# MVME-HBUT/Faster-OreFSDet

Hardware: AMD Instinct MI355X
Metric: images/sec at 640x640 25-shot (eval FPS: model(inputs) + device sync per image, bs=1 per GPU) (higher is better)
Workload: dtype f32

## Files before the change

### faster-orefsdet_amd/csrc/ore_conv_internal.h

```cpp
#pragma once
#include "ore_common.h"

namespace oreconv {

struct Lvl { int orow0, irow0, H, W, Ho, Wo; };

struct ConvP {
    const float* in; int in_ld, in_coff;
    int B, Cin;
    int nlev; Lvl lv[4];
    const float* w;
    int Cout, Cout16, kh, kw, stride, pad, M, K;
    const float* scale; const float* shift; int ep_stride; int relu_cout;
    const float* in_mul; const float* in_add; int in_relu;
    const float* add; int add_ld, add_coff, add_H, add_W;
    float* out; int out_ld, out_coff;
    float* colsum;
    int splitk, steps_per_split, nchunks;
    float* ws; int* tile_cnt;
    int bf16;
    int xmap;
    int sb;
    const float* wino;
    size_t w_lstride;
// ... 69 lines not shown
    int kw_force[4] = {};
    int gs_force[2] = {};
    int gs_ns = 3;
    int xmap_force = -1;
    int kw_nw_force = 0;
    int wino_mode = 1;
    int ws_sb_mode = 1;
    int ws_s2_mode = 1;
    int rf_mode = 1;
    int rf_force[3] = {};
    int kd_mode = 1;
    int kd_force[4] = {};
    int gd_mode = 1;
    int gd_force[3] = {};
    int gd_dbg = 0;
    int igemm[5] = {};
};
extern ConvKnobs g_knobs;

using ConvPlan = ore_conv_plan_t;
ConvPlan conv_plan(const ConvP& p, int req_splitk, size_t workspace_floats);
bool conv_wino_covers(int Cout, int Cin);
int wino_level_blocks(const ConvP& p, int gy, int* blk0);

int launch_ws(const ConvP& p, const ConvPlan& pl, hipStream_t st);
int launch_patch(const ConvP& p, const ConvPlan& pl, hipStream_t st);
int launch_igemm(const ConvP& p, const ConvPlan& pl, hipStream_t st);
int launch_wino(const ConvP& p, const ConvPlan& pl, hipStream_t st);
int launch_gd(const ConvP& p, const ConvPlan& pl, hipStream_t st);
int launch_kd(const ConvP& p, const ConvPlan& pl, hipStream_t st);
// ... 10 lines not shown
```

### faster-orefsdet_amd/csrc/ore_conv_plan.cpp

```cpp
#include "ore_common.h"
#include "ore_conv_internal.h"

namespace oreconv {

ConvKnobs g_knobs;

namespace {

const ConvKnobs& K = g_knobs;

ConvPlan make_plan(int launcher, int bm, int bn, int b0, int b1, int b2, int b3, int gx, int gy, int xmap = 0, int splitk = 1, int sps = 0) {
    ConvPlan pl{};
    pl.launcher = launcher; pl.error = ORE_OK;
    pl.bm = bm; pl.bn = bn;
    pl.build[0] = b0; pl.build[1] = b1; pl.build[2] = b2; pl.build[3] = b3;
    pl.splitk = splitk; pl.steps_per_split = sps; pl.xmap = xmap;
    pl.gx = gx; pl.gy = gy;
    return pl;
}

ConvPlan none() { return ConvPlan{}; }

ConvPlan fail(int code) {
    ConvPlan pl{};
// ... 83 lines not shown
    if (c.kh != 3 || c.kw != 3 || c.stride != 1 || c.pad != 1 || c.in_mul || c.add || c.colsum) return none();
    if (c.Cout != c.Cout16 || !conv_wino_covers(c.Cout, c.Cin)) return none();
    if (c.out_ld % 4 != 0 || c.out_coff % 4 != 0 || ((uintptr_t)c.out & 15) != 0 || c.in_ld % 4 != 0 || c.in_coff % 4 != 0) return none();
    if (c.ep_stride % 4 != 0 || ((uintptr_t)c.scale & 15) != 0 || ((uintptr_t)c.shift & 15) != 0) return none();
    if (K.wino_mode != 2 && !c.wino_lstride && c.M < ((c.Cin == 64 || c.Cin == 128) ? 1500 : 3000)) return none();
    for (int l = 0; l < c.nlev; ++l)
        if ((long long)c.lv[l].H * c.lv[l].W * c.in_ld * 4 >= (long long)kOOB) return none();
    const int nb = patch_tiles(c, 4);
    if (nb >= (1 << 22)) return none();
    if (c.Cin == 80 || c.Cin == 96 || c.Cin == 112) {
        const int ncgb = c.Cin == 80 ? 3 : 2;
        const int gy = ceil_div(c.Cout16 / 16, ncgb);
        int gx = 256 / gy;
        if (gx > nb) gx = nb;
        if (gx < 1) gx = 1;
        return make_plan(ORE_LAUNCH_WINO_NU, 4, ncgb * 16, c.Cin, ncgb, 0, 0, gx, gy);
    }
    const int coutb = c.Cin == 64 ? 64 : 32;
    const int gy = c.Cout / coutb;
    int gx = 256 / gy;
    if (gx > nb) gx = nb;
    if (gx < 1) gx = 1;
    if (c.wino_lstride) gx = wino_level_blocks(c, gy, nullptr);
    return make_plan(ORE_LAUNCH_WINO, 4, coutb, c.Cin, 0, 0, 0, gx, gy);
}

bool gd_flat(const ConvP& p) { return p.nlev > 1 && p.kh == 1 && p.kw == 1 && p.stride == 1 && p.pad == 0; }

bool gd_applies(const ConvP& p) {
    if (p.sb || p.in_mul || p.in_add || p.in_relu || (p.nlev != 1 && !gd_flat(p)) || p.ep_stride || (p.add && p.nlev != 1)) return false;
    if (p.Cin % 16 != 0 || p.in_ld % 16 != 0 || p.kh != p.kw || (p.kh != 1 && p.kh != 3)) return false;
    if (p.M >= (1 << 22) || p.nchunks > kGdTab) return false;
    const long long in_rows = gd_flat(p) ? (long long)p.lv[0].irow0 + p.M : (long long)p.lv[0].irow0 + (long long)p.B * p.lv[0].H * p.lv[0].W;
    if (in_rows * p.in_ld * 4 >= (long long)kOOB - (1 << 24) || (long long)p.Cout16 * p.K * 4 >= (long long)kOOB) return false;
    if (p.add && (long long)p.B * p.add_H * p.add_W * p.add_ld * 4 >= (long long)kOOB) return false;
    return true;
}
// ... 309 lines not shown
    return fail(ORE_EINVAL);
}

}

bool conv_wino_covers(int Cout, int Cin) {
    if (Cout <= 0 || Cout % 16 != 0) return false;
    if (Cin == 64) return Cout % 64 == 0;
    if (Cin == 128) return Cout % 32 == 0;
    return Cin == 80 || Cin == 96 || Cin == 112;
}

int wino_level_blocks(const ConvP& c, int gy, int* blk0) {
    int nb[4];
    for (int l = 0; l < c.nlev; ++l) nb[l] = c.B * ceil_div(c.lv[l].W, 16) * ceil_div(c.lv[l].H, 4);
    const int G = 256 / gy > c.nlev ? 256 / gy : c.nlev;
    int R = 1;
    for (;; ++R) {
        int need = 0;
        for (int l = 0; l < c.nlev; ++l) need += ceil_div(nb[l], R);
        if (need <= G) break;
    }
    int gx = 0;
    for (int l = 0; l < c.nlev; ++l) { if (blk0) blk0[l] = gx; gx += ceil_div(nb[l], R); }
    if (blk0) blk0[c.nlev] = gx;
    return gx;
}

ConvPlan conv_plan(const ConvP& p, int req_splitk, size_t workspace_floats) {
    ConvPlan pl;
    if (p.w_lstride) {
// ... 37 lines not shown
    case -1: k.patch_mode = BN; k.igemm[0] = 0; break;
    case -2: k.kw_mode = BN; k.igemm[0] = 0; break;
    case -3: k.kw_force[0] = BN; k.kw_force[1] = WGM; k.kw_force[2] = WGN; k.kw_force[3] = WGK; break;
    case -4: k.gs_force[0] = BN; k.gs_force[1] = WGM; if (WGN > 0) k.gs_ns = WGN; break;
    case -5: k.xmap_force = BN; break;
    case -6: k.kw_nw_force = BN; break;
    case -7: k.wino_mode = BN; break;
    case -8: k.ws_sb_mode = BN; break;
    case -9: k.ws_s2_mode = BN; break;
    case -10: k.rf_mode = BN; break;
    case -11: k.rf_force[0] = BN; k.rf_force[1] = WGM; k.rf_force[2] = WGN; break;
    case -12: k.kd_mode = BN; break;
    case -13: k.kd_force[0] = BN; k.kd_force[1] = WGM; k.kd_force[2] = WGN; k.kd_force[3] = WGK; break;
    case -14: k.gd_mode = BN; break;
    case -15: k.gd_force[0] = BN; k.gd_force[1] = WGM; k.gd_force[2] = WGN; break;
    case -16: k.gd_dbg = BN; break;
    default: k.igemm[0] = BM; k.igemm[1] = BN; k.igemm[2] = WGM; k.igemm[3] = WGN; k.igemm[4] = WGK; break;
    }
    return ORE_OK;
}

extern "C" int ore_conv_reset_plan_overrides(void) {
    g_knobs = ConvKnobs{};
    return ORE_OK;
}
```

### faster-orefsdet_amd/csrc/ore_conv_wino.hip

```cpp
#include "ore_conv_desc.h"
#include "ore_conv_epilogue.h"
#include <algorithm>

namespace {
using namespace oreconv;

struct WinoP {
    const float* in; int in_ld, in_coff;
    int B, nlev; Lvl lv[4]; int bat0[5]; int nbx[4], nby[4];
    float inv_per[4], inv_nbx[4];
    const float* U; int Cout, Cout16;
    size_t u_lstride; int blk0[5];
    const float* scale; const float* shift; int ep_stride, relu_cout;
    float* out; int out_ld, out_coff;
    int nbat;
};

struct WinoImg { __amdgpu_buffer_rsrc_t rs; unsigned pix_bytes, row_bytes; int H, W; };
__device__ __forceinline__ WinoImg wino_image(const WinoP& p, int irow0, int H, int W, int b) {
    WinoImg im;
    im.pix_bytes = (unsigned)p.in_ld * 4u; im.row_bytes = (unsigned)W * im.pix_bytes; im.H = H; im.W = W;
    im.rs = make_rsrc(p.in + ((long long)irow0 + (long long)b * (H * W)) * p.in_ld, (unsigned)H * im.row_bytes);
    return im;
}
template <int NR>
__device__ __forceinline__ void wino_patch(const WinoImg& im, int iy0, int ix0, unsigned chan_bytes, f32x4 (&d)[NR][4]) {
    unsigned cv[4], rv[NR];
#pragma unroll
    for (int c = 0; c < 4; ++c) cv[c] = (unsigned)(ix0 + c) < (unsigned)im.W ? (unsigned)(ix0 + c) * im.pix_bytes + chan_bytes : kOOB;
#pragma unroll
// ... 40 lines not shown
        t[1][b] = 0.5f * ((g[0][b] + g[2][b]) + g[1][b]);
        t[2][b] = 0.5f * ((g[0][b] + g[2][b]) - g[1][b]);
        t[3][b] = g[2][b];
    }
#pragma unroll
    for (int xi = 0; xi < 4; ++xi) {
        const float u0 = t[xi][0], u3 = t[xi][2];
        const float u1 = 0.5f * ((t[xi][0] + t[xi][2]) + t[xi][1]);
        const float u2 = 0.5f * ((t[xi][0] + t[xi][2]) - t[xi][1]);
        const float u[4] = {u0, u1, u2, u3};
#pragma unroll
        for (int nu = 0; nu < 4; ++nu) U[wino_u_index(xi * 4 + nu, n, c, Cout16, Cin)] = u[nu];
    }
}

template <int CIN>
__global__ __launch_bounds__(512, 2) void k_conv3x3_wino(WinoP p) {
    constexpr int KH = CIN / 64;
    constexpr int COUTB = 64 / KH;
    constexpr int QV = CIN / 4, QZ = COUTB / 4;
    constexpr int VF = 16 * 16 * CIN;
    static_assert(CIN == 64 || CIN == 128, "one 64-channel weight slice per wave");
    extern __shared__ __attribute__((aligned(16))) float wl[];
    float* V = wl;
    float* Z = wl + VF;
    const int tid = threadIdx.x, lane = tid & 63, w = tid >> 6;
    const int li = lane & 15, g = lane >> 4;
    const int xi = w & 3, hi = w >> 2;
    const int cb = KH == 1 ? hi * 32 : 0;
    const int cin_w0 = KH == 2 ? hi * 64 : 0;
    auto zs = [](int t) -> int { return QZ == 16 ? (t & 7) : ((t >> 1) & 3); };

    int set_s0 = 0, set_s1 = gridDim.x, set_b0 = 0, set_b1 = p.nbat;
    const float* Ub = p.U;
    if (p.u_lstride) {
        int lb = 0;
#pragma unroll
        for (int l = 1; l < 4; ++l)
            if (l < p.nlev && (int)blockIdx.x >= p.blk0[l]) lb = l;
        Ub += lb * p.u_lstride;
        set_s0 = p.blk0[lb]; set_s1 = p.blk0[lb + 1]; set_b0 = p.bat0[lb]; set_b1 = p.bat0[lb + 1];
    }
    int bat_first, bat_end;
    {
        auto below = [](int n, int c) { return (n - c + 7) >> 3; };
        const int lin0 = blockIdx.y * gridDim.x;
        const int x = (lin0 + (int)blockIdx.x) & 7;
        int v = 0;
        for (int c = 0; c < 8; ++c) {
            const int cc = (c - lin0) & 7;
            const int n_c = below(set_s1, cc) - below(set_s0, cc);
            if (c < x) v += n_c;
        }
        v += below((int)blockIdx.x, (x - lin0) & 7) - below(set_s0, (x - lin0) & 7);
        const int n = set_s1 - set_s0, cnt = set_b1 - set_b0;
        bat_first = set_b0 + (int)(((long long)v * cnt) / n);
        bat_end = set_b0 + (int)(((long long)(v + 1) * cnt) / n);
    }
    constexpr int bat_step = 1;
    f32x4 wf[4][2][4];
#pragma unroll
    for (int nu = 0; nu < 4; ++nu)
#pragma unroll
        for (int cg = 0; cg < 2; ++cg) {
            const int n16 = (blockIdx.y * COUTB + cb) / 16 + cg;
#pragma unroll
            for (int c = 0; c < 4; ++c) wf[nu][cg][c] = wino_u_frag(Ub, xi * 4 + nu, n16, (cin_w0 >> 4) + c, p.Cout16, CIN, lane);
        }

    const int q1 = tid % QV, t1 = (tid / QV) & 15;
    constexpr int NR = CIN == 64 ? 3 : 4;
    const int h1 = CIN == 64 ? __builtin_amdgcn_readfirstlane(tid >> 8) : 0;
    const int ty1 = t1 >> 3, tx1 = t1 & 7;
// ... 4 lines not shown

    int lvl = 0;
#pragma unroll
    for (int l = 1; l < 4; ++l)
        if (l < p.nlev && bat_first >= p.bat0[l]) lvl = l;
    int H = p.lv[lvl].H, W = p.lv[lvl].W, irow0 = p.lv[lvl].irow0, orow0 = p.lv[lvl].orow0, nbx = p.nbx[lvl], nby = p.nby[lvl];
    int b, byi, bxi;
    {
        const int r0 = bat_first - p.bat0[lvl], per = nbx * nby;
        b = r0 / per;
        const int r1 = r0 - b * per;
        byi = r1 / nbx; bxi = r1 - byi * nbx;
    }

    for (int bat = bat_first; bat < bat_end; bat += bat_step) {
        {
            const WinoImg im = wino_image(p, irow0, H, W, b);
            f32x4 d[NR][4];
            wino_patch<NR>(im, (byi * 2 + ty1) * 2 - 1 + h1, (bxi * 8 + tx1) * 2 - 1, chan1, d);
            float* vrow = V + t1 * CIN + ((q1 ^ t1) << 2);
            f32x4 X[4];
            if constexpr (CIN == 64) {
                if (h1 == 0) {
#pragma unroll
                    for (int c = 0; c < 4; ++c) X[c] = d[0][c] - d[2][c];
                    wino_v_store(vrow, 16 * CIN, X);
#pragma unroll
                    for (int c = 0; c < 4; ++c) X[c] = d[2][c] - d[1][c];
                    wino_v_store(vrow + (2 * 4) * 16 * CIN, 16 * CIN, X);
                } else {
#pragma unroll
                    for (int c = 0; c < 4; ++c) X[c] = d[0][c] + d[1][c];
                    wino_v_store(vrow + (1 * 4) * 16 * CIN, 16 * CIN, X);
#pragma unroll
                    for (int c = 0; c < 4; ++c) X[c] = d[0][c] - d[2][c];
                    wino_v_store(vrow + (3 * 4) * 16 * CIN, 16 * CIN, X);
                }
            } else {
#pragma unroll
                for (int x1 = 0; x1 < 4; ++x1) {
#pragma unroll
                    for (int c = 0; c < 4; ++c)
                        X[c] = x1 == 0 ? d[0][c] - d[2][c] : x1 == 1 ? d[1][c] + d[2][c] : x1 == 2 ? d[2][c] - d[1][c] : d[1][c] - d[3][c];
                    wino_v_store(vrow + (x1 * 4) * 16 * CIN, 16 * CIN, X);
                }
            }
        }
        lds_barrier();
        {
            f32x4 acc[4][2];
#pragma unroll
            for (int nu = 0; nu < 4; ++nu)
#pragma unroll
                for (int cg = 0; cg < 2; ++cg) acc[nu][cg] = f32x4{0.f, 0.f, 0.f, 0.f};
            const float* vb = V + ((xi * 4) * 16 + li) * CIN;
#pragma unroll
            for (int c = 0; c < 4; ++c) {
                const int qoff = ((((cin_w0 >> 2) + c * 4 + g) ^ li) << 2);
                f32x4 bf[4];
#pragma unroll
                for (int nu = 0; nu < 4; ++nu) bf[nu] = *reinterpret_cast<const f32x4*>(vb + nu * 16 * CIN + qoff);
#pragma unroll
                for (int nu = 0; nu < 4; ++nu)
#pragma unroll
                    for (int k = 0; k < 4; ++k)
#pragma unroll
                        for (int cg = 0; cg < 2; ++cg)
                            acc[nu][cg] = __builtin_amdgcn_mfma_f32_16x16x4f32(wf[nu][cg][c][k], bf[nu][k], acc[nu][cg], 0, 0, 0);
            }
            float* zb = Z + (((xi * KH + (KH == 2 ? hi : 0)) * 2) * 16 + li) * COUTB;
#pragma unroll
            for (int cg = 0; cg < 2; ++cg) {
                const int quad = ((cb >> 2) + cg * 4 + g) ^ zs(li);
                *reinterpret_cast<f32x4*>(zb + (quad << 2)) = (acc[0][cg] + acc[1][cg]) + acc[2][cg];
                *reinterpret_cast<f32x4*>(zb + 16 * COUTB + (quad << 2)) = (acc[1][cg] - acc[2][cg]) - acc[3][cg];
            }
        }
        lds_barrier();
        if (p3_on) {
            f32x4 z[4];
#pragma unroll
            for (int x = 0; x < 4; ++x) {
                const float* zr = Z + (((x * KH) * 2 + j3) * 16 + t3) * COUTB + ((cq3 ^ zs(t3)) << 2);
                z[x] = *reinterpret_cast<const f32x4*>(zr);
                if (KH == 2) z[x] += *reinterpret_cast<const f32x4*>(zr + 2 * 16 * COUTB);
            }
            const f32x4 y0 = (z[0] + z[1]) + z[2], y1 = (z[1] - z[2]) - z[3];
            const int n = blockIdx.y * COUTB + cq3 * 4;
            f32x4 sc, sh;
            scale_shift4_vec(p, lvl, n, sc, sh);
            f32x4 v0 = y0 * sc + sh, v1 = y1 * sc + sh;
            CONV_RELU4_X2(v0, v1, n, p.relu_cout)
            const int oy = (byi * 2 + ty3) * 2, ox = (bxi * 8 + tx3) * 2 + j3;
            if (ox < W && oy < H) {
                float* o = p.out + (size_t)(orow0 + b * H * W + oy * W + ox) * p.out_ld + p.out_coff + n;
                *reinterpret_cast<f32x4*>(o) = v0;
                if (oy + 1 < H) *reinterpret_cast<f32x4*>(o + (size_t)W * p.out_ld) = v1;
            }
        }
        if (++bxi == nbx) {
            bxi = 0;
            if (++byi == nby) {
                byi = 0;
                if (++b == p.B && bat + bat_step < bat_end) {
                    b = 0; ++lvl;
                    H = p.lv[lvl].H; W = p.lv[lvl].W; irow0 = p.lv[lvl].irow0; orow0 = p.lv[lvl].orow0; nbx = p.nbx[lvl]; nby = p.nby[lvl];
                }
            }
        }
    }
}

template <int CIN, int NCGB>
__global__ __launch_bounds__(512, 2) void k_conv3x3_wino_nu(WinoP p) {
    constexpr int NC = CIN / 16, COUTB = NCGB * 16;
    constexpr int QV = CIN / 4, QZ = COUTB / 4;
    constexpr int VS = CIN + 4, ZS = COUTB + 4;
    constexpr int VF = 16 * 16 * VS;
    static_assert(CIN % 16 == 0 && 16 * QV <= 512 && 32 * QZ <= 512, "one P1 / P3 item per thread");
    extern __shared__ __attribute__((aligned(16))) float wl[];
    float* V = wl;
    float* Z = wl + VF;
    const int tid = threadIdx.x, lane = tid & 63, w = __builtin_amdgcn_readfirstlane(threadIdx.x >> 6);
    const int li = lane & 15, g = lane >> 4;
    const int xi = w & 3, hi = w >> 2;
    const int n16_0 = blockIdx.y * NCGB, ncg_real = min(NCGB, (p.Cout16 >> 4) - n16_0);

    f32x4 wf[2][NCGB][NC];
#pragma unroll
    for (int n2 = 0; n2 < 2; ++n2)
#pragma unroll
        for (int cg = 0; cg < NCGB; ++cg)
#pragma unroll
            for (int c = 0; c < NC; ++c)
                wf[n2][cg][c] = cg < ncg_real ? wino_u_frag(p.U, xi * 4 + hi * 2 + n2, n16_0 + cg, c, p.Cout16, CIN, lane)
                                              : f32x4{0.f, 0.f, 0.f, 0.f};

    const bool p1_on = tid < 16 * QV;
    const int q1 = tid % QV, t1 = (tid / QV) & 15;
    const int ty1 = t1 >> 3, tx1 = t1 & 7;
    const int cq3 = tid % QZ, j3 = (tid / QZ) & 1, t3 = tid / (2 * QZ);
    const int n3 = blockIdx.y * COUTB + cq3 * 4;
    const bool p3_on = t3 < 16 && n3 < p.Cout;
    const int ty3 = (t3 & 15) >> 3, tx3 = t3 & 7;
    const unsigned chan1 = (unsigned)(p.in_coff + q1 * 4) * 4u;

    int lvl = 0, H = p.lv[0].H, W = p.lv[0].W, irow0 = p.lv[0].irow0, orow0 = p.lv[0].orow0, nbx = p.nbx[0], per = p.nbx[0] * p.nby[0];
    int lvl_b0 = 0, lvl_b1 = p.bat0[1];
    float inv_per = p.inv_per[0], inv_nbx = p.inv_nbx[0];
    for (int bat = blockIdx.x; bat < p.nbat; bat += gridDim.x) {
        if (bat >= lvl_b1) {
            do { ++lvl; } while (bat >= p.bat0[lvl + 1]);
            H = p.lv[lvl].H; W = p.lv[lvl].W; irow0 = p.lv[lvl].irow0; orow0 = p.lv[lvl].orow0; nbx = p.nbx[lvl]; per = nbx * p.nby[lvl];
            lvl_b0 = p.bat0[lvl]; lvl_b1 = p.bat0[lvl + 1]; inv_per = p.inv_per[lvl]; inv_nbx = p.inv_nbx[lvl];
        }
        const int r0 = bat - lvl_b0;
        const int b = fdiv(r0, per, inv_per), r1 = r0 - b * per;
        const int byi = fdiv(r1, nbx, inv_nbx), bxi = r1 - byi * nbx;
        if (p1_on) {
            const WinoImg im = wino_image(p, irow0, H, W, b);
            f32x4 d[4][4];
            wino_patch<4>(im, (byi * 2 + ty1) * 2 - 1, (bxi * 8 + tx1) * 2 - 1, chan1, d);
            float* vrow = V + t1 * VS + q1 * 4;
#pragma unroll
            for (int x1 = 0; x1 < 4; ++x1) {
                f32x4 X[4];
#pragma unroll
                for (int c = 0; c < 4; ++c)
                    X[c] = x1 == 0 ? d[0][c] - d[2][c] : x1 == 1 ? d[1][c] + d[2][c] : x1 == 2 ? d[2][c] - d[1][c] : d[1][c] - d[3][c];
                wino_v_store(vrow + (x1 * 4) * 16 * VS, 16 * VS, X);
            }
        }
        lds_barrier();
        {
            f32x4 acc[2][NCGB];
#pragma unroll
            for (int n2 = 0; n2 < 2; ++n2)
#pragma unroll
                for (int cg = 0; cg < NCGB; ++cg) acc[n2][cg] = f32x4{0.f, 0.f, 0.f, 0.f};
            const float* vb = V + ((xi * 4 + hi * 2) * 16 + li) * VS + g * 4;
#pragma unroll
            for (int c = 0; c < NC; ++c) {
                f32x4 bf[2];
#pragma unroll
                for (int n2 = 0; n2 < 2; ++n2) bf[n2] = *reinterpret_cast<const f32x4*>(vb + n2 * 16 * VS + c * 16);
#pragma unroll
                for (int k = 0; k < 4; ++k)
#pragma unroll
                    for (int n2 = 0; n2 < 2; ++n2)
#pragma unroll
                        for (int cg = 0; cg < NCGB; ++cg)
                            acc[n2][cg] = __builtin_amdgcn_mfma_f32_16x16x4f32(wf[n2][cg][c][k], bf[n2][k], acc[n2][cg], 0, 0, 0);
            }
            float* zb = Z + (((xi * 2 + hi) * 2) * 16 + li) * ZS + g * 4;
#pragma unroll
            for (int cg = 0; cg < NCGB; ++cg) {
                const f32x4 z0 = hi == 0 ? acc[0][cg] + acc[1][cg] : acc[0][cg];
                const f32x4 z1 = hi == 0 ? acc[1][cg] : -(acc[0][cg] + acc[1][cg]);
                *reinterpret_cast<f32x4*>(zb + cg * 16) = z0;
                *reinterpret_cast<f32x4*>(zb + 16 * ZS + cg * 16) = z1;
            }
        }
        lds_barrier();
        if (p3_on) {
            f32x4 z[4];
#pragma unroll
            for (int x = 0; x < 4; ++x) {
                const float* zr = Z + (((x * 2) * 2 + j3) * 16 + t3) * ZS + cq3 * 4;
                z[x] = *reinterpret_cast<const f32x4*>(zr) + *reinterpret_cast<const f32x4*>(zr + 2 * 16 * ZS);
            }
            const f32x4 y0 = (z[0] + z[1]) + z[2], y1 = (z[1] - z[2]) - z[3];
            f32x4 sc, sh;
            scale_shift4_vec(p, lvl, n3, sc, sh);
            f32x4 v0 = y0 * sc + sh, v1 = y1 * sc + sh;
            CONV_RELU4_X2(v0, v1, n3, p.relu_cout)
            const int oy = (byi * 2 + ty3) * 2, ox = (bxi * 8 + tx3) * 2 + j3;
            if (ox < W && oy < H) {
                float* o = p.out + (size_t)(orow0 + b * H * W + oy * W + ox) * p.out_ld + p.out_coff + n3;
                *reinterpret_cast<f32x4*>(o) = v0;
                if (oy + 1 < H) *reinterpret_cast<f32x4*>(o + (size_t)W * p.out_ld) = v1;
            }
        }
    }
}

template <int CIN, int NCGB>
int wino_nu_go(const WinoP& p, dim3 grid, hipStream_t st) {
    const size_t lds = ((size_t)16 * 16 * (CIN + 4) + 4 * 2 * 2 * 16 * (NCGB * 16 + 4)) * sizeof(float);
    static bool attr = false;
    if (!attr) {
        ORE_HIP(hipFuncSetAttribute((const void*)k_conv3x3_wino_nu<CIN, NCGB>, hipFuncAttributeMaxDynamicSharedMemorySize, (int)lds));
        attr = true;
    }
    hipLaunchKernelGGL((k_conv3x3_wino_nu<CIN, NCGB>), grid, dim3(512), lds, st, p);
    return ore_launch_status("k_conv3x3_wino_nu");
}

int wino_go(const ConvP& c, const WinoP& p, dim3 grid, hipStream_t st) {
    if (c.Cin == 80) return wino_nu_go<80, 3>(p, grid, st);
    if (c.Cin == 96) return wino_nu_go<96, 2>(p, grid, st);
    if (c.Cin == 112) return wino_nu_go<112, 2>(p, grid, st);
    const size_t lds = ((size_t)16 * 16 * c.Cin + 4 * 2 * 16 * 64) * sizeof(float);
    static bool attr = false;
    if (!attr) {
        ORE_HIP(hipFuncSetAttribute((const void*)k_conv3x3_wino<64>, hipFuncAttributeMaxDynamicSharedMemorySize, (int)(96 * 1024)));
        ORE_HIP(hipFuncSetAttribute((const void*)k_conv3x3_wino<128>, hipFuncAttributeMaxDynamicSharedMemorySize, (int)(160 * 1024)));
        attr = true;
    }
    if (c.Cin == 64) hipLaunchKernelGGL(k_conv3x3_wino<64>, grid, dim3(512), lds, st, p);
    else hipLaunchKernelGGL(k_conv3x3_wino<128>, grid, dim3(512), lds, st, p);
    return ore_launch_status("k_conv3x3_wino");
}

}

namespace oreconv {

int launch_wino(const ConvP& c, const ConvPlan& pl, hipStream_t st) {
    WinoP p{};
    p.in = c.in; p.in_ld = c.in_ld; p.in_coff = c.in_coff; p.B = c.B; p.nlev = c.nlev;
    int nb = 0;
    for (int l = 0; l < c.nlev; ++l) {
        p.lv[l] = c.lv[l];
        p.nbx[l] = ceil_div(c.lv[l].W, 16); p.nby[l] = ceil_div(c.lv[l].H, 4);
        p.inv_per[l] = 1.0f / (float)(p.nbx[l] * p.nby[l]); p.inv_nbx[l] = 1.0f / (float)p.nbx[l];
        p.bat0[l] = nb;
        nb += c.B * p.nbx[l] * p.nby[l];
    }
    p.bat0[c.nlev] = nb; p.nbat = nb;
    p.U = c.wino; p.Cout = c.Cout; p.Cout16 = c.Cout16;
    p.scale = c.scale; p.shift = c.shift; p.ep_stride = c.ep_stride; p.relu_cout = c.relu_cout;
    p.out = c.out; p.out_ld = c.out_ld; p.out_coff = c.out_coff;
    if (c.wino_lstride) { p.u_lstride = c.wino_lstride; wino_level_blocks(c, pl.gy, p.blk0); }
    const int rc = wino_go(c, p, dim3(pl.gx, pl.gy), st);
    if (rc == 0) ore_note_wino(1);
    return rc;
}

}

extern "C" int32_t ore_winograd_covers(int32_t Cout, int32_t Cin) { return oreconv::conv_wino_covers(Cout, Cin) ? 1 : 0; }

extern "C" size_t ore_winograd_weight_floats(int32_t Cout, int32_t Cin) { return (size_t)16 * round_up(Cout, 16) * Cin; }

extern "C" int ore_winograd_weight_fwd(const float* packed_w, int32_t Cout, int32_t Cin, float* U, void* stream) {
    ORE_CHECK_ARG(packed_w && U && Cout > 0 && Cin > 0, "ore_winograd_weight_fwd: bad args");
    const int C16 = round_up(Cout, 16), n = C16 * Cin;
    hipLaunchKernelGGL(k_wino_weight, dim3(ceil_div(n, 256)), dim3(256), 0, (hipStream_t)stream, packed_w, C16, Cin, U);
    return ore_launch_status("k_wino_weight");
// ... 2 lines not shown
```

### faster-orefsdet_amd/csrc/ore_util.cpp

```cpp
#include <stdarg.h>
#include <stdio.h>
#include "ore_hip.h"

static thread_local char g_err[512] = "";

void ore_set_error(const char* fmt, ...) {
    va_list ap;
    va_start(ap, fmt);
    vsnprintf(g_err, sizeof(g_err), fmt, ap);
    va_end(ap);
}

extern "C" const char* ore_last_error(void) { return g_err; }

#include <atomic>
static std::atomic<double> g_flops{0.0};
static std::atomic<long long> g_flop_calls{0};
void ore_flop_count_add(double flops) {
    double cur = g_flops.load(std::memory_order_relaxed);
    while (!g_flops.compare_exchange_weak(cur, cur + flops, std::memory_order_relaxed)) {}
    g_flop_calls.fetch_add(1, std::memory_order_relaxed);
}
static thread_local int g_last_wino = 0;
void ore_note_wino(int v) { g_last_wino = v; }
int ore_last_wino(void) { return g_last_wino; }
static thread_local int g_last_launch = ORE_LAUNCH_NONE, g_last_split = 1;
void ore_note_launch(int code, int split) { g_last_launch = code; g_last_split = split; }
extern "C" int32_t ore_conv_last_launch(int32_t* split) {
    if (split) *split = g_last_split;
    return g_last_launch;
}
extern "C" int ore_flop_counter_read(double* flops, int64_t* calls, int32_t reset) {
    if (flops) *flops = g_flops.load(std::memory_order_relaxed);
    if (calls) *calls = (int64_t)g_flop_calls.load(std::memory_order_relaxed);
    if (reset) { g_flops.store(0.0, std::memory_order_relaxed); g_flop_calls.store(0, std::memory_order_relaxed); }
    return ORE_OK;
}
extern "C" double ore_dwpw_flops(int64_t rows, int32_t C) { return 2.0 * (double)rows * (double)C * (9.0 + (double)C); }
extern "C" int32_t ore_det_record_rows(void) { return ORE_DET_RECORD_ROWS; }
extern "C" int ore_version(void) { return 601; }
```

### include/ore_hip.h

```cpp
#ifndef ORE_HIP_H_
#define ORE_HIP_H_
#include <stddef.h>
#include <stdint.h>
#ifdef __cplusplus
extern "C" {
#endif

#define ORE_OK 0
#define ORE_EINVAL (-22)
#define ORE_ENOMEM (-12)
#define ORE_EHIP (-5)
#define ORE_ENOENT (-2)

const char* ore_last_error(void);
int ore_version(void);
int ore_flop_counter_read(double* flops, int64_t* calls, int32_t reset);


typedef struct ore_conv_desc {
    const float* in;   int32_t in_ld, in_coff;
    int32_t B, H, W, Cin;
    const float* w;
    int32_t Cout, kh, kw, stride, pad;
    const float* scale;
// ... 17 lines not shown
#define ORE_ST_BF16_F32OUT 2
size_t ore_packed_weight_bf16_elems(int32_t Cout, int32_t Cin, int32_t kh, int32_t kw);
int ore_pack_conv_weight_bf16_host(const float* w_oihw, int32_t Cout, int32_t Cin, int32_t kh, int32_t kw, uint16_t* dst);

int32_t ore_winograd_covers(int32_t Cout, int32_t Cin);
size_t ore_winograd_weight_floats(int32_t Cout, int32_t Cin);
int ore_winograd_weight_fwd(const float* packed_w, int32_t Cout, int32_t Cin, float* U, void* stream);

#define ORE_CONV_CNT_INTS 4096
#define ORE_CONV_WS_FLOATS ((size_t)ORE_CONV_CNT_INTS + ((size_t)8 << 20))
size_t ore_conv_workspace_floats(void);
int32_t ore_conv_colsum_rows(const ore_conv_desc* d);

int ore_conv2d_fwd(const ore_conv_desc* d, void* stream);
int ore_conv_set_plan_override(int32_t BM, int32_t BN, int32_t WGM, int32_t WGN, int32_t WGK);
#define ORE_LAUNCH_NONE 0
#define ORE_LAUNCH_WINO 1
#define ORE_LAUNCH_WINO_NU 2
#define ORE_LAUNCH_GD 3
#define ORE_LAUNCH_PATCH4 4
#define ORE_LAUNCH_PATCH8 5
#define ORE_LAUNCH_PATCH_DB 6
#define ORE_LAUNCH_WS64 7
#define ORE_LAUNCH_WS128 8
#define ORE_LAUNCH_KD 9
#define ORE_LAUNCH_RF 10
#define ORE_LAUNCH_GS 11
#define ORE_LAUNCH_KW 12
#define ORE_LAUNCH_IGEMM 13
#define ORE_LAUNCH_WS_SB 14
// ... 539 lines not shown
```

Baseline: 1689.

## Split Winograd tail batches into half-Cout units to balance block load

Adds a work-dealing scheme for the Winograd conv kernels. When the last round of batches would leave blocks idle, the remaining batches are split into half-output-channel units spread across more blocks. For the non-uniform Cout kernel, blocks can also be redistributed between full and partial channel-group rows. This targets tail imbalance in the final round. It adds TAIL template variants, larger code size and some register pressure, and only engages when the cost heuristic says splitting pays.

Measured after the change: 1703 (median of 6 runs). No clear change (+0.8%).

```diff
diff --git a/faster-orefsdet_amd/csrc/ore_conv_internal.h b/faster-orefsdet_amd/csrc/ore_conv_internal.h
--- a/faster-orefsdet_amd/csrc/ore_conv_internal.h
+++ b/faster-orefsdet_amd/csrc/ore_conv_internal.h
@@ -107,6 +107,7 @@
     int gd_mode = 1;
     int gd_force[3] = {};
     int gd_dbg = 0;
+    int wino_deal[2] = {1, 0};
     int igemm[5] = {};
 };
 extern ConvKnobs g_knobs;
diff --git a/faster-orefsdet_amd/csrc/ore_conv_plan.cpp b/faster-orefsdet_amd/csrc/ore_conv_plan.cpp
--- a/faster-orefsdet_amd/csrc/ore_conv_plan.cpp
+++ b/faster-orefsdet_amd/csrc/ore_conv_plan.cpp
@@ -1,5 +1,6 @@
 #include "ore_common.h"
 #include "ore_conv_internal.h"
+#include "ore_wino_deal.h"
 
 namespace oreconv {
 
@@ -121,6 +122,7 @@
         int gx = 256 / gy;
         if (gx > nb) gx = nb;
         if (gx < 1) gx = 1;
+        if (K.wino_deal[1] > 0 && gx > K.wino_deal[1]) gx = K.wino_deal[1];
         return make_plan(ORE_LAUNCH_WINO_NU, 4, ncgb * 16, c.Cin, ncgb, 0, 0, gx, gy);
     }
     const int coutb = c.Cin == 64 ? 64 : 32;
@@ -128,6 +130,7 @@
     int gx = 256 / gy;
     if (gx > nb) gx = nb;
     if (gx < 1) gx = 1;
+    if (K.wino_deal[1] > 0 && gx > K.wino_deal[1]) gx = K.wino_deal[1];
     if (c.wino_lstride) gx = wino_level_blocks(c, gy, nullptr);
     return make_plan(ORE_LAUNCH_WINO, 4, coutb, c.Cin, 0, 0, 0, gx, gy);
 }
@@ -467,7 +470,9 @@
 int wino_level_blocks(const ConvP& c, int gy, int* blk0) {
     int nb[4];
     for (int l = 0; l < c.nlev; ++l) nb[l] = c.B * ceil_div(c.lv[l].W, 16) * ceil_div(c.lv[l].H, 4);
-    const int G = 256 / gy > c.nlev ? 256 / gy : c.nlev;
+    int G = 256 / gy;
+    if (g_knobs.wino_deal[1] > 0 && G > g_knobs.wino_deal[1]) G = g_knobs.wino_deal[1];
+    if (G < c.nlev) G = c.nlev;
     int R = 1;
     for (;; ++R) {
         int need = 0;
@@ -535,8 +540,24 @@
     case -13: k.kd_force[0] = BN; k.kd_force[1] = WGM; k.kd_force[2] = WGN; k.kd_force[3] = WGK; break;
     case -14: k.gd_mode = BN; break;
     case -15: k.gd_force[0] = BN; k.gd_force[1] = WGM; k.gd_force[2] = WGN; break;
+    case -17: k.wino_deal[0] = BN; k.wino_deal[1] = WGM; break;
     case -16: k.gd_dbg = BN; break;
     default: k.igemm[0] = BM; k.igemm[1] = BN; k.igemm[2] = WGM; k.igemm[3] = WGN; k.igemm[4] = WGK; break;
+    }
+    return ORE_OK;
+}
+
+extern "C" int ore_wino_deal_query(int32_t gx, int32_t gy, int32_t cnt, int32_t ncgb, int32_t ncg_last, int32_t* out) {
+    ORE_CHECK_ARG(out && gx > 0 && gy > 0 && cnt >= 0 && (ncgb == 0 || (ncgb >= 2 && ncgb <= 3 && ncg_last >= 1 && ncg_last <= ncgb)),
+                  "ore_wino_deal_query: bad args");
+    const int split = g_knobs.wino_deal[0] != 0;
+    int nf = gx, whole[2] = {cnt, cnt};
+    const bool tail = ncgb ? wino_nu_deal(gx, gy, cnt, ncgb, ncg_last, split, nf, whole) : wino_tail_pays(1, &gx, &cnt, split);
+    for (int lin = 0; lin < gx * gy; ++lin, out += 8) {
+        const WinoRow r = wino_nu_row(lin, gx, gy, nf);
+        const WinoDeal d = wino_deal(r.rank, r.G, cnt, ncgb ? whole[r.row == gy - 1] < cnt : tail, ncgb != 0);
+        out[0] = r.row; out[1] = r.rank; out[2] = r.G; out[3] = d.first; out[4] = d.nfull; out[5] = ncgb ? r.G : 1;
+        out[6] = d.half_bat; out[7] = d.half_cg;
     }
     return ORE_OK;
 }
diff --git a/faster-orefsdet_amd/csrc/ore_conv_wino.hip b/faster-orefsdet_amd/csrc/ore_conv_wino.hip
--- a/faster-orefsdet_amd/csrc/ore_conv_wino.hip
+++ b/faster-orefsdet_amd/csrc/ore_conv_wino.hip
@@ -1,6 +1,8 @@
 #include "ore_conv_desc.h"
 #include "ore_conv_epilogue.h"
+#include "ore_wino_deal.h"
 #include <algorithm>
+#include <type_traits>
 
 namespace {
 using namespace oreconv;
@@ -14,6 +16,8 @@
     const float* scale; const float* shift; int ep_stride, relu_cout;
     float* out; int out_ld, out_coff;
     int nbat;
+    int nu_nf;
+    int nu_whole[2];
 };
 
 struct WinoImg { __amdgpu_buffer_rsrc_t rs; unsigned pix_bytes, row_bytes; int H, W; };
@@ -84,7 +88,7 @@
     }
 }
 
-template <int CIN>
+template <int CIN, bool TAIL>
 __global__ __launch_bounds__(512, 2) void k_conv3x3_wino(WinoP p) {
     constexpr int KH = CIN / 64;
     constexpr int COUTB = 64 / KH;
@@ -111,7 +115,7 @@
         Ub += lb * p.u_lstride;
         set_s0 = p.blk0[lb]; set_s1 = p.blk0[lb + 1]; set_b0 = p.bat0[lb]; set_b1 = p.bat0[lb + 1];
     }
-    int bat_first, bat_end;
+    WinoDeal deal;
     {
         auto below = [](int n, int c) { return (n - c + 7) >> 3; };
         const int lin0 = blockIdx.y * gridDim.x;
@@ -123,10 +127,9 @@
             if (c < x) v += n_c;
         }
         v += below((int)blockIdx.x, (x - lin0) & 7) - below(set_s0, (x - lin0) & 7);
-        const int n = set_s1 - set_s0, cnt = set_b1 - set_b0;
-        bat_first = set_b0 + (int)(((long long)v * cnt) / n);
-        bat_end = set_b0 + (int)(((long long)(v + 1) * cnt) / n);
-    }
+        deal = wino_deal(v, set_s1 - set_s0, set_b1 - set_b0, TAIL ? 1 : 0, 0);
+    }
+    const int bat_first = set_b0 + deal.first, bat_end = bat_first + deal.nfull;
     constexpr int bat_step = 1;
     f32x4 wf[4][2][4];
 #pragma unroll
@@ -161,90 +164,9 @@
     }
 
     for (int bat = bat_first; bat < bat_end; bat += bat_step) {
-        {
-            const WinoImg im = wino_image(p, irow0, H, W, b);
-            f32x4 d[NR][4];
-            wino_patch<NR>(im, (byi * 2 + ty1) * 2 - 1 + h1, (bxi * 8 + tx1) * 2 - 1, chan1, d);
-            float* vrow = V + t1 * CIN + ((q1 ^ t1) << 2);
-            f32x4 X[4];
-            if constexpr (CIN == 64) {
-                if (h1 == 0) {
-#pragma unroll
-                    for (int c = 0; c < 4; ++c) X[c] = d[0][c] - d[2][c];
-                    wino_v_store(vrow, 16 * CIN, X);
-#pragma unroll
-                    for (int c = 0; c < 4; ++c) X[c] = d[2][c] - d[1][c];
-                    wino_v_store(vrow + (2 * 4) * 16 * CIN, 16 * CIN, X);
-                } else {
-#pragma unroll
-                    for (int c = 0; c < 4; ++c) X[c] = d[0][c] + d[1][c];
-                    wino_v_store(vrow + (1 * 4) * 16 * CIN, 16 * CIN, X);
-#pragma unroll
-                    for (int c = 0; c < 4; ++c) X[c] = d[0][c] - d[2][c];
-                    wino_v_store(vrow + (3 * 4) * 16 * CIN, 16 * CIN, X);
-                }
-            } else {
-#pragma unroll
-                for (int x1 = 0; x1 < 4; ++x1) {
-#pragma unroll
-                    for (int c = 0; c < 4; ++c)
-                        X[c] = x1 == 0 ? d[0][c] - d[2][c] : x1 == 1 ? d[1][c] + d[2][c] : x1 == 2 ? d[2][c] - d[1][c] : d[1][c] - d[3][c];
-                    wino_v_store(vrow + (x1 * 4) * 16 * CIN, 16 * CIN, X);
-                }
-            }
-        }
-        lds_barrier();
-        {
-            f32x4 acc[4][2];
-#pragma unroll
-            for (int nu = 0; nu < 4; ++nu)
-#pragma unroll
-                for (int cg = 0; cg < 2; ++cg) acc[nu][cg] = f32x4{0.f, 0.f, 0.f, 0.f};
-            const float* vb = V + ((xi * 4) * 16 + li) * CIN;
-#pragma unroll
-            for (int c = 0; c < 4; ++c) {
-                const int qoff = ((((cin_w0 >> 2) + c * 4 + g) ^ li) << 2);
-                f32x4 bf[4];
-#pragma unroll
-                for (int nu = 0; nu < 4; ++nu) bf[nu] = *reinterpret_cast<const f32x4*>(vb + nu * 16 * CIN + qoff);
-#pragma unroll
-                for (int nu = 0; nu < 4; ++nu)
-#pragma unroll
-                    for (int k = 0; k < 4; ++k)
-#pragma unroll
-                        for (int cg = 0; cg < 2; ++cg)
-                            acc[nu][cg] = __builtin_amdgcn_mfma_f32_16x16x4f32(wf[nu][cg][c][k], bf[nu][k], acc[nu][cg], 0, 0, 0);
-            }
-            float* zb = Z + (((xi * KH + (KH == 2 ? hi : 0)) * 2) * 16 + li) * COUTB;
-#pragma unroll
-            for (int cg = 0; cg < 2; ++cg) {
-                const int quad = ((cb >> 2) + cg * 4 + g) ^ zs(li);
-                *reinterpret_cast<f32x4*>(zb + (quad << 2)) = (acc[0][cg] + acc[1][cg]) + acc[2][cg];
-                *reinterpret_cast<f32x4*>(zb + 16 * COUTB + (quad << 2)) = (acc[1][cg] - acc[2][cg]) - acc[3][cg];
-            }
-        }
-        lds_barrier();
-        if (p3_on) {
-            f32x4 z[4];
-#pragma unroll
-            for (int x = 0; x < 4; ++x) {
-                const float* zr = Z + (((x * KH) * 2 + j3) * 16 + t3) * COUTB + ((cq3 ^ zs(t3)) << 2);
-                z[x] = *reinterpret_cast<const f32x4*>(zr);
-                if (KH == 2) z[x] += *reinterpret_cast<const f32x4*>(zr + 2 * 16 * COUTB);
-            }
-            const f32x4 y0 = (z[0] + z[1]) + z[2], y1 = (z[1] - z[2]) - z[3];
-            const int n = blockIdx.y * COUTB + cq3 * 4;
-            f32x4 sc, sh;
-            scale_shift4_vec(p, lvl, n, sc, sh);
-            f32x4 v0 = y0 * sc + sh, v1 = y1 * sc + sh;
-            CONV_RELU4_X2(v0, v1, n, p.relu_cout)
-            const int oy = (byi * 2 + ty3) * 2, ox = (bxi * 8 + tx3) * 2 + j3;
-            if (ox < W && oy < H) {
-                float* o = p.out + (size_t)(orow0 + b * H * W + oy * W + ox) * p.out_ld + p.out_coff + n;
-                *reinterpret_cast<f32x4*>(o) = v0;
-                if (oy + 1 < H) *reinterpret_cast<f32x4*>(o + (size_t)W * p.out_ld) = v1;
-            }
-        }
+#define WINO_HC (-1)
+#include "ore_conv_wino_unit.inc"
+#undef WINO_HC
         if (++bxi == nbx) {
             bxi = 0;
             if (++byi == nby) {
@@ -256,9 +178,30 @@
             }
         }
     }
-}
-
-template <int CIN, int NCGB>
+    if (TAIL && deal.half_bat >= 0) {
+        const int hb = set_b0 + deal.half_bat;
+        lvl = 0;
+#pragma unroll
+        for (int l = 1; l < 4; ++l)
+            if (l < p.nlev && hb >= p.bat0[l]) lvl = l;
+        H = p.lv[lvl].H; W = p.lv[lvl].W; irow0 = p.lv[lvl].irow0; orow0 = p.lv[lvl].orow0; nbx = p.nbx[lvl]; nby = p.nby[lvl];
+        const int r0 = hb - p.bat0[lvl], per = nbx * nby;
+        b = r0 / per;
+        const int r1 = r0 - b * per;
+        byi = r1 / nbx; bxi = r1 - byi * nbx;
+        if (deal.half_cg == 0) {
+#define WINO_HC 0
+#include "ore_conv_wino_unit.inc"
+#undef WINO_HC
+        } else {
+#define WINO_HC 1
+#include "ore_conv_wino_unit.inc"
+#undef WINO_HC
+        }
+    }
+}
+
+template <int CIN, int NCGB, bool TAIL>
 __global__ __launch_bounds__(512, 2) void k_conv3x3_wino_nu(WinoP p) {
     constexpr int NC = CIN / 16, COUTB = NCGB * 16;
     constexpr int QV = CIN / 4, QZ = COUTB / 4;
@@ -271,7 +214,9 @@
     const int tid = threadIdx.x, lane = tid & 63, w = __builtin_amdgcn_readfirstlane(threadIdx.x >> 6);
     const int li = lane & 15, g = lane >> 4;
     const int xi = w & 3, hi = w >> 2;
-    const int n16_0 = blockIdx.y * NCGB, ncg_real = min(NCGB, (p.Cout16 >> 4) - n16_0);
+    WinoRow br{(int)blockIdx.y, (int)blockIdx.x, (int)gridDim.x};
+    if (TAIL && p.nu_nf != (int)gridDim.x) br = wino_nu_row(blockIdx.y * gridDim.x + blockIdx.x, gridDim.x, gridDim.y, p.nu_nf);
+    const int n16_0 = br.row * NCGB, ncg_real = min(NCGB, (p.Cout16 >> 4) - n16_0);
 
     f32x4 wf[2][NCGB][NC];
 #pragma unroll
@@ -287,7 +232,7 @@
     const int q1 = tid % QV, t1 = (tid / QV) & 15;
     const int ty1 = t1 >> 3, tx1 = t1 & 7;
     const int cq3 = tid % QZ, j3 = (tid / QZ) & 1, t3 = tid / (2 * QZ);
-    const int n3 = blockIdx.y * COUTB + cq3 * 4;
+    const int n3 = br.row * COUTB + cq3 * 4;
     const bool p3_on = t3 < 16 && n3 < p.Cout;
     const int ty3 = (t3 & 15) >> 3, tx3 = t3 & 7;
     const unsigned chan1 = (unsigned)(p.in_coff + q1 * 4) * 4u;
@@ -295,7 +240,9 @@
     int lvl = 0, H = p.lv[0].H, W = p.lv[0].W, irow0 = p.lv[0].irow0, orow0 = p.lv[0].orow0, nbx = p.nbx[0], per = p.nbx[0] * p.nby[0];
     int lvl_b0 = 0, lvl_b1 = p.bat0[1];
     float inv_per = p.inv_per[0], inv_nbx = p.inv_nbx[0];
-    for (int bat = blockIdx.x; bat < p.nbat; bat += gridDim.x) {
+    const int whole = TAIL ? p.nu_whole[br.row == (int)gridDim.y - 1 ? 1 : 0] : p.nbat;
+    auto unit = [&](auto ng_tag, auto c0_tag, const int bat) __attribute__((always_inline)) {
+        constexpr int NG = decltype(ng_tag)::value, C0 = decltype(c0_tag)::value;
         if (bat >= lvl_b1) {
             do { ++lvl; } while (bat >= p.bat0[lvl + 1]);
             H = p.lv[lvl].H; W = p.lv[lvl].W; irow0 = p.lv[lvl].irow0; orow0 = p.lv[lvl].orow0; nbx = p.nbx[lvl]; per = nbx * p.nby[lvl];
@@ -324,7 +271,7 @@
 #pragma unroll
             for (int n2 = 0; n2 < 2; ++n2)
 #pragma unroll
-                for (int cg = 0; cg < NCGB; ++cg) acc[n2][cg] = f32x4{0.f, 0.f, 0.f, 0.f};
+                for (int cg = C0; cg < C0 + NG; ++cg) acc[n2][cg] = f32x4{0.f, 0.f, 0.f, 0.f};
             const float* vb = V + ((xi * 4 + hi * 2) * 16 + li) * VS + g * 4;
 #pragma unroll
             for (int c = 0; c < NC; ++c) {
@@ -336,12 +283,12 @@
 #pragma unroll
                     for (int n2 = 0; n2 < 2; ++n2)
 #pragma unroll
-                        for (int cg = 0; cg < NCGB; ++cg)
-                            acc[n2][cg] = __builtin_amdgcn_mfma_f32_16x16x4f32(wf[n2][cg][c][k], bf[n2][k], acc[n2][cg], 0, 0, 0);
+                        for (int cg = C0; cg < C0 + NG; ++cg)
+                            acc[n2][cg] =__builtin_amdgcn_mfma_f32_16x16x4f32(wf[n2][cg][c][k], bf[n2][k], acc[n2][cg], 0, 0, 0);
             }
             float* zb = Z + (((xi * 2 + hi) * 2) * 16 + li) * ZS + g * 4;
 #pragma unroll
-            for (int cg = 0; cg < NCGB; ++cg) {
+            for (int cg = C0; cg < C0 + NG; ++cg) {
                 const f32x4 z0 = hi == 0 ? acc[0][cg] + acc[1][cg] : acc[0][cg];
                 const f32x4 z1 = hi == 0 ? acc[1][cg] : -(acc[0][cg] + acc[1][cg]);
                 *reinterpret_cast<f32x4*>(zb + cg * 16) = z0;
@@ -349,7 +296,7 @@
             }
         }
         lds_barrier();
-        if (p3_on) {
+        if (NG == NCGB ? p3_on : p3_on && (unsigned)((cq3 >> 2) - C0) < (unsigned)NG) {
             f32x4 z[4];
 #pragma unroll
             for (int x = 0; x < 4; ++x) {
@@ -368,34 +315,50 @@
                 if (oy + 1 < H) *reinterpret_cast<f32x4*>(o + (size_t)W * p.out_ld) = v1;
             }
         }
-    }
-}
-
-template <int CIN, int NCGB>
+    };
+    auto walk = [&](auto ng_tag) __attribute__((always_inline)) {
+        for (int bat = br.rank; bat < whole; bat += br.G) unit(ng_tag, std::integral_constant<int, 0>{}, bat);
+    };
+    if (!TAIL || ncg_real == NCGB) walk(std::integral_constant<int, NCGB>{});
+    else if (ncg_real == NCGB - 1) walk(std::integral_constant<int, NCGB - 1>{});
+    else if constexpr (NCGB == 3) walk(std::integral_constant<int, 1>{});
+    int half_bat, half_cg;
+    wino_half(br.rank, br.G, p.nbat, whole, half_bat, half_cg);
+    if (TAIL && half_bat >= 0) {
+        if (half_cg == 0) unit(std::integral_constant<int, 1>{}, std::integral_constant<int, 0>{}, half_bat);
+        else unit(std::integral_constant<int, 1>{}, std::integral_constant<int, 1>{}, half_bat);
+    }
+}
+
+template <int CIN, int NCGB, bool TAIL>
 int wino_nu_go(const WinoP& p, dim3 grid, hipStream_t st) {
     const size_t lds = ((size_t)16 * 16 * (CIN + 4) + 4 * 2 * 2 * 16 * (NCGB * 16 + 4)) * sizeof(float);
     static bool attr = false;
     if (!attr) {
-        ORE_HIP(hipFuncSetAttribute((const void*)k_conv3x3_wino_nu<CIN, NCGB>, hipFuncAttributeMaxDynamicSharedMemorySize, (int)lds));
+        ORE_HIP(hipFuncSetAttribute((const void*)k_conv3x3_wino_nu<CIN, NCGB, TAIL>, hipFuncAttributeMaxDynamicSharedMemorySize, (int)lds));
         attr = true;
     }
-    hipLaunchKernelGGL((k_conv3x3_wino_nu<CIN, NCGB>), grid, dim3(512), lds, st, p);
+    hipLaunchKernelGGL((k_conv3x3_wino_nu<CIN, NCGB, TAIL>), grid, dim3(512), lds, st, p);
     return ore_launch_status("k_conv3x3_wino_nu");
 }
 
-int wino_go(const ConvP& c, const WinoP& p, dim3 grid, hipStream_t st) {
-    if (c.Cin == 80) return wino_nu_go<80, 3>(p, grid, st);
-    if (c.Cin == 96) return wino_nu_go<96, 2>(p, grid, st);
-    if (c.Cin == 112) return wino_nu_go<112, 2>(p, grid, st);
+int wino_go(const ConvP& c, const WinoP& p, bool tail, dim3 grid, hipStream_t st) {
+    if (c.Cin == 80) return tail ? wino_nu_go<80, 3, true>(p, grid, st) : wino_nu_go<80, 3, false>(p, grid, st);
+    if (c.Cin == 96) return tail ? wino_nu_go<96, 2, true>(p, grid, st) : wino_nu_go<96, 2, false>(p, grid, st);
+    if (c.Cin == 112) return tail ? wino_nu_go<112, 2, true>(p, grid, st) : wino_nu_go<112, 2, false>(p, grid, st);
     const size_t lds = ((size_t)16 * 16 * c.Cin + 4 * 2 * 16 * 64) * sizeof(float);
     static bool attr = false;
     if (!attr) {
-        ORE_HIP(hipFuncSetAttribute((const void*)k_conv3x3_wino<64>, hipFuncAttributeMaxDynamicSharedMemorySize, (int)(96 * 1024)));
-        ORE_HIP(hipFuncSetAttribute((const void*)k_conv3x3_wino<128>, hipFuncAttributeMaxDynamicSharedMemorySize, (int)(160 * 1024)));
+        ORE_HIP(hipFuncSetAttribute((const void*)k_conv3x3_wino<64, false>, hipFuncAttributeMaxDynamicSharedMemorySize, (int)(96 * 1024)));
+        ORE_HIP(hipFuncSetAttribute((const void*)k_conv3x3_wino<64, true>, hipFuncAttributeMaxDynamicSharedMemorySize, (int)(96 * 1024)));
+        ORE_HIP(hipFuncSetAttribute((const void*)k_conv3x3_wino<128, false>, hipFuncAttributeMaxDynamicSharedMemorySize, (int)(160 * 1024)));
+        ORE_HIP(hipFuncSetAttribute((const void*)k_conv3x3_wino<128, true>, hipFuncAttributeMaxDynamicSharedMemorySize, (int)(160 * 1024)));
         attr = true;
     }
-    if (c.Cin == 64) hipLaunchKernelGGL(k_conv3x3_wino<64>, grid, dim3(512), lds, st, p);
-    else hipLaunchKernelGGL(k_conv3x3_wino<128>, grid, dim3(512), lds, st, p);
+    if (c.Cin == 64 && tail) hipLaunchKernelGGL((k_conv3x3_wino<64, true>), grid, dim3(512), lds, st, p);
+    else if (c.Cin == 64) hipLaunchKernelGGL((k_conv3x3_wino<64, false>), grid, dim3(512), lds, st, p);
+    else if (tail) hipLaunchKernelGGL((k_conv3x3_wino<128, true>), grid, dim3(512), lds, st, p);
+    else hipLaunchKernelGGL((k_conv3x3_wino<128, false>), grid, dim3(512), lds, st, p);
     return ore_launch_status("k_conv3x3_wino");
 }
 
@@ -419,7 +382,20 @@
     p.scale = c.scale; p.shift = c.shift; p.ep_stride = c.ep_stride; p.relu_cout = c.relu_cout;
     p.out = c.out; p.out_ld = c.out_ld; p.out_coff = c.out_coff;
     if (c.wino_lstride) { p.u_lstride = c.wino_lstride; wino_level_blocks(c, pl.gy, p.blk0); }
-    const int rc = wino_go(c, p, dim3(pl.gx, pl.gy), st);
+    const int split = g_knobs.wino_deal[0] != 0;
+    bool tail;
+    p.nu_nf = pl.gx;
+    if (pl.launcher == ORE_LAUNCH_WINO_NU) {
+        const int ncgb = pl.build[1], ncg_last = c.Cout16 / 16 - (pl.gy - 1) * ncgb;
+        tail = wino_nu_deal(pl.gx, pl.gy, nb, ncgb, ncg_last, split, p.nu_nf, p.nu_whole);
+    } else if (p.u_lstride) {
+        int G[4], cnt[4];
+        for (int l = 0; l < c.nlev; ++l) { G[l] = p.blk0[l + 1] - p.blk0[l]; cnt[l] = p.bat0[l + 1] - p.bat0[l]; }
+        tail = wino_tail_pays(c.nlev, G, cnt, split);
+    } else {
+        tail = wino_tail_pays(1, &pl.gx, &nb, split);
+    }
+    const int rc = wino_go(c, p, tail, dim3(pl.gx, pl.gy), st);
     if (rc == 0) ore_note_wino(1);
     return rc;
 }
diff --git a/faster-orefsdet_amd/csrc/ore_conv_wino_unit.inc b/faster-orefsdet_amd/csrc/ore_conv_wino_unit.inc
--- /dev/null
+++ b/faster-orefsdet_amd/csrc/ore_conv_wino_unit.inc
@@ -0,0 +1,97 @@
+{
+        constexpr int HC = WINO_HC;
+        constexpr bool HALF = HC >= 0;
+        constexpr int CG0 = HALF ? HC : 0, CG1 = HALF ? HC + 1 : 2;
+        {
+            const WinoImg im = wino_image(p, irow0, H, W, b);
+            f32x4 d[NR][4];
+            wino_patch<NR>(im, (byi * 2 + ty1) * 2 - 1 + h1, (bxi * 8 + tx1) * 2 - 1, chan1, d);
+            float* vrow = V + t1 * CIN + ((q1 ^ t1) << 2);
+            f32x4 X[4];
+            if constexpr (CIN == 64) {
+                if (h1 == 0) {
+#pragma unroll
+                    for (int c = 0; c < 4; ++c) X[c] = d[0][c] - d[2][c];
+                    wino_v_store(vrow, 16 * CIN, X);
+#pragma unroll
+                    for (int c = 0; c < 4; ++c) X[c] = d[2][c] - d[1][c];
+                    wino_v_store(vrow + (2 * 4) * 16 * CIN, 16 * CIN, X);
+                } else {
+#pragma unroll
+                    for (int c = 0; c < 4; ++c) X[c] = d[0][c] + d[1][c];
+                    wino_v_store(vrow + (1 * 4) * 16 * CIN, 16 * CIN, X);
+#pragma unroll
+                    for (int c = 0; c < 4; ++c) X[c] = d[0][c] - d[2][c];
+                    wino_v_store(vrow + (3 * 4) * 16 * CIN, 16 * CIN, X);
+                }
+            } else {
+#pragma unroll
+                for (int x1 = 0; x1 < 4; ++x1) {
+#pragma unroll
+                    for (int c = 0; c < 4; ++c)
+                        X[c] = x1 == 0 ? d[0][c] - d[2][c] : x1 == 1 ? d[1][c] + d[2][c] : x1 == 2 ? d[2][c] - d[1][c] : d[1][c] - d[3][c];
+                    wino_v_store(vrow + (x1 * 4) * 16 * CIN, 16 * CIN, X);
+                }
+            }
+        }
+        lds_barrier();
+        {
+            f32x4 acc[4][2];
+#pragma unroll
+            for (int nu = 0; nu < 4; ++nu)
+#pragma unroll
+                for (int cg = CG0; cg < CG1; ++cg) acc[nu][cg] = f32x4{0.f, 0.f, 0.f, 0.f};
+            const float* vb = V + ((xi * 4) * 16 + li) * CIN;
+#pragma unroll
+            for (int c = 0; c < 4; ++c) {
+                const int qoff = ((((cin_w0 >> 2) + c * 4 + g) ^ li) << 2);
+                f32x4 bf[4];
+#pragma unroll
+                for (int nu = 0; nu < 4; ++nu) bf[nu] = *reinterpret_cast<const f32x4*>(vb + nu * 16 * CIN + qoff);
+#pragma unroll
+                for (int nu = 0; nu < 4; ++nu)
+#pragma unroll
+                    for (int k = 0; k < 4; ++k)
+#pragma unroll
+                        for (int cg = CG0; cg < CG1; ++cg)
+                            acc[nu][cg] = __builtin_amdgcn_mfma_f32_16x16x4f32(wf[nu][cg][c][k], bf[nu][k], acc[nu][cg], 0, 0, 0);
+            }
+            float* zb = Z + (((xi * KH + (KH == 2 ? hi : 0)) * 2) * 16 + li) * COUTB;
+#pragma unroll
+            for (int cg = CG0; cg < CG1; ++cg) {
+                const int quad = ((cb >> 2) + cg * 4 + g) ^ zs(li);
+                *reinterpret_cast<f32x4*>(zb + (quad << 2)) = (acc[0][cg] + acc[1][cg]) + acc[2][cg];
+                *reinterpret_cast<f32x4*>(zb + 16 * COUTB + (quad << 2)) = (acc[1][cg] - acc[2][cg]) - acc[3][cg];
+            }
+        }
+        lds_barrier();
+        int pt = t3, pj = j3, pq = cq3, pty = ty3, ptx = tx3;
+        bool pon = p3_on;
+        if constexpr (HALF) {
+            const int qh = tid % (QZ / 2);
+            pq = KH == 1 ? (qh >> 2) * 8 + HC * 4 + (qh & 3) : HC * 4 + qh;
+            pj = (tid / (QZ / 2)) & 1; pt = tid / QZ; pon = pt < 16;
+            pty = (pt & 15) >> 3; ptx = pt & 7;
+        }
+        if (pon) {
+            f32x4 z[4];
+#pragma unroll
+            for (int x = 0; x < 4; ++x) {
+                const float* zr = Z + (((x * KH) * 2 + pj) * 16 + pt) * COUTB + ((pq ^ zs(pt)) << 2);
+                z[x] = *reinterpret_cast<const f32x4*>(zr);
+                if (KH == 2) z[x] += *reinterpret_cast<const f32x4*>(zr + 2 * 16 * COUTB);
+            }
+            const f32x4 y0 = (z[0] + z[1]) + z[2], y1 = (z[1] - z[2]) - z[3];
+            const int n = blockIdx.y * COUTB + pq * 4;
+            f32x4 sc, sh;
+            scale_shift4_vec(p, lvl, n, sc, sh);
+            f32x4 v0 = y0 * sc + sh, v1 = y1 * sc + sh;
+            CONV_RELU4_X2(v0, v1, n, p.relu_cout)
+            const int oy = (byi * 2 + pty) * 2, ox = (bxi * 8 + ptx) * 2 + pj;
+            if (ox < W && oy < H) {
+                float* o = p.out + (size_t)(orow0 + b * H * W + oy * W + ox) * p.out_ld + p.out_coff + n;
+                *reinterpret_cast<f32x4*>(o) = v0;
+                if (oy + 1 < H) *reinterpret_cast<f32x4*>(o + (size_t)W * p.out_ld) = v1;
+            }
+        }
+}
diff --git a/faster-orefsdet_amd/csrc/ore_util.cpp b/faster-orefsdet_amd/csrc/ore_util.cpp
--- a/faster-orefsdet_amd/csrc/ore_util.cpp
+++ b/faster-orefsdet_amd/csrc/ore_util.cpp
@@ -38,4 +38,4 @@
 }
 extern "C" double ore_dwpw_flops(int64_t rows, int32_t C) { return 2.0 * (double)rows * (double)C * (9.0 + (double)C); }
 extern "C" int32_t ore_det_record_rows(void) { return ORE_DET_RECORD_ROWS; }
-extern "C" int ore_version(void) { return 601; }
+extern "C" int ore_version(void) { return 602; }
diff --git a/faster-orefsdet_amd/csrc/ore_wino_deal.h b/faster-orefsdet_amd/csrc/ore_wino_deal.h
--- /dev/null
+++ b/faster-orefsdet_amd/csrc/ore_wino_deal.h
@@ -0,0 +1,91 @@
+#pragma once
+
+#if defined(__HIPCC__)
+#define ORE_WINO_HD __host__ __device__
+#else
+#define ORE_WINO_HD
+#endif
+
+namespace oreconv {
+
+struct WinoDeal {
+    int first, nfull;
+    int half_bat, half_cg;
+};
+
+constexpr int kWinoTailMaxRounds = 8;
+ORE_WINO_HD inline bool wino_tail_pays(int nsets, const int* G, const int* cnt, int split) {
+    if (!split) return false;
+    int maxr = 0;
+    for (int s = 0; s < nsets; ++s) { const int r = (cnt[s] + G[s] - 1) / G[s]; if (r > maxr) maxr = r; }
+    if (maxr > kWinoTailMaxRounds) return false;
+    for (int s = 0; s < nsets; ++s) {
+        const int R = cnt[s] / G[s], L = cnt[s] - R * G[s];
+        if (R + (L > 0) == maxr && !(L > 0 && 2 * L <= G[s])) return false;
+    }
+    return true;
+}
+
+ORE_WINO_HD inline int wino_whole(int G, int cnt, int split) {
+    const int R = cnt / G, L = cnt - R * G;
+    return split && L > 0 && 2 * L <= G ? G * R : cnt;
+}
+ORE_WINO_HD inline void wino_half(int rank, int G, int cnt, int whole, int& half_bat, int& half_cg) {
+    const int h = rank - (G - 2 * (cnt - whole));
+    half_bat = whole < cnt && h >= 0 ? whole + (h >> 1) : -1;
+    half_cg = half_bat >= 0 ? h & 1 : 0;
+}
+
+ORE_WINO_HD inline WinoDeal wino_deal(int rank, int G, int cnt, int split, int strided) {
+    WinoDeal d;
+    const int R = cnt / G, L = cnt - R * G, whole = wino_whole(G, cnt, split);
+    wino_half(rank, G, cnt, whole, d.half_bat, d.half_cg);
+    if (whole < cnt) {
+        d.first = strided ? rank : rank * R;
+        d.nfull = R;
+    } else if (strided) {
+        d.first = rank;
+        d.nfull = R + (rank < L ? 1 : 0);
+    } else {
+        d.first = (int)(((long long)rank * cnt) / G);
+        d.nfull = (int)(((long long)(rank + 1) * cnt) / G) - d.first;
+    }
+    return d;
+}
+
+ORE_WINO_HD inline int wino_nu_full_blocks(int gx, int gy, int cnt, int ncgb, int ncg_last, int split) {
+    if (!split || gy < 2 || ncg_last >= ncgb) return gx;
+    const int T = gx * gy, uf = 3 * ncgb, us = ncgb + 2 * ncg_last;
+    const int r_now = (cnt + gx - 1) / gx;
+    if (r_now > kWinoTailMaxRounds) return gx;
+    int best = gx, best_cost = r_now * uf;
+    for (int rf = 1; rf < r_now; ++rf) {
+        const int nf = (cnt + rf - 1) / rf, ns = T - (gy - 1) * nf;
+        if (ns < 1) continue;
+        const int rs = (cnt + ns - 1) / ns;
+        const int cost = rf * uf > rs * us ? rf * uf : rs * us;
+        if (cost < best_cost) { best = nf; best_cost = cost; }
+    }
+    return best;
+}
+
+ORE_WINO_HD inline bool wino_nu_deal(int gx, int gy, int cnt, int ncgb, int ncg_last, int split, int& nf, int* whole) {
+    nf = wino_nu_full_blocks(gx, gy, cnt, ncgb, ncg_last, split);
+    const int ns = gx * gy - (gy - 1) * nf;
+    const bool few = (cnt + gx - 1) / gx <= kWinoTailMaxRounds;
+    whole[0] = wino_whole(nf, cnt, split && few && ncgb == 2);
+    whole[1] = wino_whole(ns, cnt, split && few && ncg_last == 2);
+    return nf != gx || whole[0] < cnt || whole[1] < cnt;
+}
+
+struct WinoRow { int row, rank, G; };
+ORE_WINO_HD inline WinoRow wino_nu_row(int lin, int gx, int gy, int nf) {
+    WinoRow r;
+    r.row = lin / nf;
+    if (r.row > gy - 1) r.row = gy - 1;
+    r.rank = lin - r.row * nf;
+    r.G = r.row < gy - 1 ? nf : gx * gy - (gy - 1) * nf;
+    return r;
+}
+
+}
diff --git a/include/ore_hip.h b/include/ore_hip.h
--- a/include/ore_hip.h
+++ b/include/ore_hip.h
@@ -55,6 +55,7 @@
 
 int ore_conv2d_fwd(const ore_conv_desc* d, void* stream);
 int ore_conv_set_plan_override(int32_t BM, int32_t BN, int32_t WGM, int32_t WGN, int32_t WGK);
+int ore_wino_deal_query(int32_t gx, int32_t gy, int32_t cnt, int32_t ncgb, int32_t ncg_last, int32_t* out);
 #define ORE_LAUNCH_NONE 0
 #define ORE_LAUNCH_WINO 1
 #define ORE_LAUNCH_WINO_NU 2
```
